# hangxu0304/DeepReduce

Hardware: NVIDIA H100
Metric: ResNet-50 images/sec (whole job, device-timed, max over ranks) (higher is better)
Workload: dtype bf16

## Files before the change

deepreduce_b200/ops/csrc/binding.cpp:

```cpp
#include <ATen/cuda/CUDAContext.h>
#include <c10/cuda/CUDAGuard.h>
#include <c10/cuda/CUDAStream.h>
#include <torch/extension.h>

#include <condition_variable>
#include <deque>
#include <mutex>
#include <thread>

#include "ops.h"

namespace py = pybind11;
using dr::EngineParams;

#define CHECK_CUDA_T(x) TORCH_CHECK((x).is_cuda() && (x).is_contiguous(), #x " must be a contiguous CUDA tensor")

static cudaStream_t cur_stream() { return at::cuda::getCurrentCUDAStream().stream(); }

static void check_last(const char* what) {
  cudaError_t e = cudaGetLastError();
  TORCH_CHECK(e == cudaSuccess, what, ": ", cudaGetErrorString(e));
}

static torch::Tensor bloom_insert(torch::Tensor idx, int64_t k, int64_t m_bits, int64_t seed) {
// ... 144 lines not shown
  const int64_t nb = (n + 127) / 128;
  auto off = torch::empty({nb + 1}, payload.options().dtype(torch::kInt64));
  auto deltas = torch::empty({n}, payload.options().dtype(torch::kInt64));
  dr::launch_bp128_unpack((const uint32_t*)payload.data_ptr<int32_t>(), n, off.data_ptr<int64_t>(),
                          deltas.data_ptr<int64_t>(), cur_stream());
  check_last("delta_bp128_decode");
  return deltas.cumsum(0);
}

static torch::Tensor rle_runs(torch::Tensor idx, int64_t d) {
  CHECK_CUDA_T(idx);
  c10::cuda::CUDAGuard g(idx.device());
  const int64_t n = idx.numel();
  auto o64 = idx.options().dtype(torch::kInt64);
  if (n == 0) return torch::full({1}, d, o64);
  const int64_t nb = (n + 1023) / 1024;
  auto counts = torch::empty({nb}, idx.options().dtype(torch::kInt32));
  auto excl = torch::empty({nb + 1}, idx.options().dtype(torch::kInt32));
  dr::launch_rle_count(idx.data_ptr<int64_t>(), n, (uint32_t*)counts.data_ptr<int32_t>(), (uint32_t*)excl.data_ptr<int32_t>(),
                       cur_stream());
  const int64_t n_runs = excl[nb].item<int32_t>();
  auto start_pos = torch::empty({n_runs}, o64), end_pos = torch::empty({n_runs}, o64);
  auto runs = torch::zeros({2 * n_runs + 1}, o64);
  dr::launch_rle_runs(idx.data_ptr<int64_t>(), n, (const uint32_t*)excl.data_ptr<int32_t>(), start_pos.data_ptr<int64_t>(),
                      end_pos.data_ptr<int64_t>(), n_runs, d, runs.data_ptr<int64_t>(), cur_stream());
  check_last("rle_runs");
  const int64_t last = idx[n - 1].item<int64_t>();
  return (d - 1 - last > 0) ? runs : runs.slice(0, 0, 2 * n_runs);
}

static torch::Tensor rle_indices(torch::Tensor runs) {
  CHECK_CUDA_T(runs);
  c10::cuda::CUDAGuard g(runs.device());
  const int64_t n_pairs = runs.numel() / 2;
  auto o64 = runs.options().dtype(torch::kInt64);
  if (n_pairs == 0) return torch::empty({0}, o64);
  auto pairs = runs.slice(0, 0, 2 * n_pairs).to(torch::kInt64).view({n_pairs, 2});
  auto z = pairs.select(1, 0), o = pairs.select(1, 1);
  auto csum = (z + o).cumsum(0);
  auto run_start = (csum - o).contiguous();
  auto ones_incl = o.cumsum(0);
  auto ones_excl = (ones_incl - o).contiguous();
  const int64_t total = ones_incl[n_pairs - 1].item<int64_t>();
  auto out = torch::empty({total}, o64);
  dr::launch_rle_expand(ones_excl.data_ptr<int64_t>(), run_start.data_ptr<int64_t>(), n_pairs, total, out.data_ptr<int64_t>(),
                        cur_stream());
  check_last("rle_indices");
  return out;
}

static torch::Tensor u8_to_nhwc_norm(torch::Tensor in, std::vector<double> mean, std::vector<double> stdv) {
  CHECK_CUDA_T(in);
  TORCH_CHECK(in.scalar_type() == torch::kUInt8 && in.size(-1) == 3, "expect uint8 [...,3] NHWC");
  c10::cuda::CUDAGuard g(in.device());
  auto out = torch::empty(in.sizes(), in.options().dtype(torch::kBFloat16));
  float m[3] = {(float)mean[0], (float)mean[1], (float)mean[2]};
  float s[3] = {(float)(1.0 / stdv[0]), (float)(1.0 / stdv[1]), (float)(1.0 / stdv[2])};
  dr::launch_u8_to_nhwc_norm(in.data_ptr<uint8_t>(), out.data_ptr(), in.numel() / 3, m, s, cur_stream());
  check_last("u8_to_nhwc_norm");
  return out;
}

namespace at::native {
struct Var;
template <typename scalar_t, typename VarTransform>
void batch_norm_stats_channels_last_cuda_template(const at::Tensor& out_mean, const at::Tensor& out_invstd,
                                                   const at::Tensor& input, double epsilon);
}

static void check_bn_input(const torch::Tensor& x) {
  TORCH_CHECK(x.is_cuda() && x.scalar_type() == torch::kBFloat16 && x.dim() == 4 && x.stride(1) == 1 &&
                  x.is_contiguous(at::MemoryFormat::ChannelsLast),
              "bn: x must be a channels_last bf16 CUDA tensor");
  TORCH_CHECK(x.size(1) % 8 == 0 && x.size(1) <= 8192, "bn: channels must be a multiple of 8, at most 8192");
  TORCH_CHECK(x.numel() < std::numeric_limits<int32_t>::max(), "bn: tensor too large for 32-bit indexing");
}

static void check_chan(const torch::Tensor& t, int64_t C, const char* what) {
  TORCH_CHECK(t.is_cuda() && t.scalar_type() == torch::kFloat32 && t.is_contiguous() && t.numel() == C, "bn: ", what,
              " must be a contiguous float32 CUDA tensor of C elements");
}

static std::vector<torch::Tensor> bn_stats(torch::Tensor x, torch::Tensor running_mean, torch::Tensor running_var,
                                           double momentum, double eps) {
  check_bn_input(x);
  const int64_t C = x.size(1);
  check_chan(running_mean, C, "running_mean");
  check_chan(running_var, C, "running_var");
  const int64_t N = x.numel() / C;
  TORCH_CHECK(N > 1, "bn: expected more than 1 value per channel when training");
  c10::cuda::CUDAGuard g(x.device());
  auto opts = x.options().dtype(torch::kFloat32);
  auto mean = torch::empty({C}, opts), var = torch::empty({C}, opts);
  at::native::batch_norm_stats_channels_last_cuda_template<c10::BFloat16, at::native::Var>(mean, var, x, eps);
  const float bessel = static_cast<float>(static_cast<double>(N) / static_cast<double>(N - 1));
  cudaError_t e = dr::launch_bn_update_stats(mean.data_ptr<float>(), var.data_ptr<float>(), running_mean.data_ptr<float>(),
                                             running_var.data_ptr<float>(), (int)C, (float)momentum, bessel, (float)eps,
                                             cur_stream());
  TORCH_CHECK(e == cudaSuccess, "bn_stats: ", cudaGetErrorString(e));
  return {mean, var};
}

static dr::BnParams bn_params(const std::vector<torch::Tensor>& p, int64_t C) {
  TORCH_CHECK(p.size() == 4, "bn: expected (mean, invstd, weight, bias)");
  const char* names[4] = {"mean", "invstd", "weight", "bias"};
  for (int i = 0; i < 4; ++i) check_chan(p[i], C, names[i]);
  return {p[0].data_ptr<float>(), p[1].data_ptr<float>(), p[2].data_ptr<float>(), p[3].data_ptr<float>()};
}

static void check_like_x(const torch::Tensor& t, const torch::Tensor& x, const char* what) {
  TORCH_CHECK(t.sizes() == x.sizes() && t.strides() == x.strides() && t.scalar_type() == torch::kBFloat16 &&
                  t.device() == x.device(),
              "bn: ", what, " must match x in shape, layout, dtype and device");
}

static std::vector<torch::Tensor> bn_apply(int64_t mode, torch::Tensor x, std::vector<torch::Tensor> p,
                                           c10::optional<torch::Tensor> z, std::vector<torch::Tensor> pz) {
  check_bn_input(x);
  const int64_t C = x.size(1);
  const dr::BnParams px = bn_params(p, C);
  dr::BnParams pzz{};
  const void* zp = nullptr;
  if (mode != 0) {
    TORCH_CHECK(z.has_value(), "bn: mode ", mode, " needs z");
    check_like_x(*z, x, "z");
    zp = z->data_ptr();
    if (mode == 2) pzz = bn_params(pz, C);
  }
  c10::cuda::CUDAGuard g(x.device());
  const int64_t rows = x.numel() / C;
  auto out = torch::empty_like(x);
  auto mask = torch::empty({rows, C / 8}, x.options().dtype(torch::kUInt8));
  cudaError_t e = dr::launch_bn_apply((int)mode, x.data_ptr(), px, zp, pzz, out.data_ptr(), mask.data_ptr(), rows,
                                      (int)C, cur_stream());
  TORCH_CHECK(e == cudaSuccess, "bn_apply: ", cudaGetErrorString(e));
  return {out, mask};
}

static dr::BnParams bn_bwd_params(const std::vector<torch::Tensor>& p, int64_t C) {
  TORCH_CHECK(p.size() == 3, "bn_backward: expected (mean, invstd, weight)");
  const char* names[3] = {"mean", "invstd", "weight"};
  for (int i = 0; i < 3; ++i) check_chan(p[i], C, names[i]);
  return {p[0].data_ptr<float>(), p[1].data_ptr<float>(), p[2].data_ptr<float>(), nullptr};
}

static std::vector<torch::Tensor> bn_backward(int64_t mode, torch::Tensor go, torch::Tensor mask, torch::Tensor x,
                                              std::vector<torch::Tensor> p, c10::optional<torch::Tensor> z,
                                              std::vector<torch::Tensor> pz) {
  TORCH_CHECK(mode >= 0 && mode <= 2, "bn_backward: mode must be 0, 1 or 2");
  check_bn_input(x);
  TORCH_CHECK(go.sizes() == x.sizes() && go.scalar_type() == torch::kBFloat16 && go.device() == x.device() &&
                  go.is_contiguous(at::MemoryFormat::ChannelsLast),
              "bn_backward: go must be a channels_last bf16 tensor of x's shape on x's device");
  const int64_t C = x.size(1), rows = x.numel() / C;
  TORCH_CHECK(mask.is_cuda() && mask.scalar_type() == torch::kUInt8 && mask.is_contiguous() &&
                  mask.numel() == rows * (C / 8) && mask.device() == x.device(),
              "bn_backward: mask must be bn_apply's mask for x");
  c10::cuda::CUDAGuard guard(x.device());
  int block_y = 0, grid_y = 0;
  dr::bn_backward_tree(rows, (int)C, &block_y, &grid_y);
  TORCH_CHECK((int64_t)block_y * grid_y <= rows, "bn_backward: reduction tree wider than the rows");
  const int n_sums = mode == 2 ? 3 : 2;
  auto f32 = x.options().dtype(torch::kFloat32);
  auto sums = torch::empty({n_sums, C}, f32);
  auto staging = grid_y > 1 ? torch::empty({n_sums, grid_y, C}, f32) : torch::Tensor();
  auto dx = torch::empty_like(x), dw = torch::empty({C}, f32), db = torch::empty({C}, f32);
  dr::BnBwd b{};
  b.go = go.data_ptr(); b.mask = mask.data_ptr<uint8_t>(); b.x = x.data_ptr();
  b.px = bn_bwd_params(p, C);
  b.dx = dx.data_ptr(); b.sums = sums.data_ptr<float>(); b.staging = grid_y > 1 ? staging.data_ptr<float>() : nullptr;
  b.dw = dw.data_ptr<float>(); b.db = db.data_ptr<float>();
  std::vector<torch::Tensor> res{dx, dw, db};
  if (mode == 1) {
    auto g = torch::empty_like(x);
    b.g = g.data_ptr();
    res.push_back(g);
  } else if (mode == 2) {
    TORCH_CHECK(z.has_value(), "bn_backward: mode 2 needs z");
    check_like_x(*z, x, "z");
    b.z = z->data_ptr();
    b.pz = bn_bwd_params(pz, C);
    auto dz = torch::empty_like(x), dwz = torch::empty({C}, f32), dbz = torch::empty({C}, f32);
    b.dz = dz.data_ptr(); b.dwz = dwz.data_ptr<float>(); b.dbz = dbz.data_ptr<float>();
    res.insert(res.end(), {dz, dwz, dbz});
  }
  cudaError_t e = dr::launch_bn_backward((int)mode, b, rows, (int)C, cur_stream());
  TORCH_CHECK(e == cudaSuccess, "bn_backward: ", cudaGetErrorString(e));
  return res;
}

struct Engine {
  EngineParams P{};
  int grid = 0;
  int grid_cap = 0;
  int blocks_per_sm = 2;
  int dyn_smem = 64 * 1024;
  int device = 0;

  Engine(int64_t tensors, int64_t tiles, int64_t n_tensors, int64_t n_tiles, int64_t slot_words,
         int64_t payload_words, int64_t grad, int64_t resid, int64_t hist, int64_t hist_total, int64_t sel,
         int64_t tile_count, int64_t barrier, int64_t status, std::vector<int64_t> arenas, int rank, int world) {
    TORCH_CHECK(world <= dr::kMaxWorld && (int)arenas.size() == world, "bad world/arenas");
    P.tensors = reinterpret_cast<const dr::TensorDesc*>(tensors);
    P.tiles = reinterpret_cast<const dr::TileInfo*>(tiles);
    P.n_tensors = (uint32_t)n_tensors; P.n_tiles = (uint32_t)n_tiles;
    P.slot_words = (uint32_t)slot_words; P.payload_words = (uint32_t)payload_words;
    P.grad = reinterpret_cast<float*>(grad); P.resid = reinterpret_cast<float*>(resid);
    P.hist = reinterpret_cast<uint32_t*>(hist); P.hist_total = reinterpret_cast<uint32_t*>(hist_total);
    P.sel = reinterpret_cast<dr::SelState*>(sel);
    P.tile_count = reinterpret_cast<uint32_t*>(tile_count);
    P.barrier = reinterpret_cast<uint32_t*>(barrier); P.status = reinterpret_cast<uint32_t*>(status);
    for (int i = 0; i < world; ++i) P.arena[i] = reinterpret_cast<uint32_t*>(arenas[i]);
    P.rank = rank; P.world = world;
    P.beta = 1.f; P.gamma = 1.f; P.scale = 1.f / world; P.seed = dr::kDefaultSeed; P.policy = 0; P.use_history = 1;
    P.spin_limit = 20u * 1000u * 1000u;
    P.filter_smem_words = (uint32_t)(dyn_smem / 4);
    P.use_tma = 1; P.hist_shift = 23;
    P.shard = 0; P.s2_words = 0; P.s2_cap = 0; P.has_rle = 0; P.mc_arena = nullptr;
    P.peer_timeout_ms = 120000u; P.fault = 0; P.debug_times = nullptr; P.cost_prefix = nullptr; P.deterministic = 0; P.cuts = nullptr; P.cuts_grid = 0;
    cudaGetDevice(&device);
  }

  void configure(double beta, double gamma, double scale, int64_t seed, int policy, int use_history, int64_t spin_limit,
                 int bps, int64_t filter_smem_bytes, int use_tma, int hist_shift) {
    P.beta = (float)beta; P.gamma = (float)gamma; P.scale = (float)scale; P.seed = (uint32_t)seed;
    P.policy = policy; P.use_history = use_history; P.spin_limit = (uint32_t)spin_limit;
    blocks_per_sm = bps; grid = 0;
    dyn_smem = (int)filter_smem_bytes; P.filter_smem_words = (uint32_t)(dyn_smem / 4);
    P.use_tma = use_tma; P.hist_shift = (uint32_t)hist_shift;
  }

  void set_poly(int64_t tensors, int64_t n_poly, int64_t tasks, int64_t n_tasks, int64_t bins, int64_t bucket_val,
                int64_t bucket_pos, int64_t expand_buf, int64_t poly_total) {
    P.poly_tensors = reinterpret_cast<const uint32_t*>(tensors); P.n_poly = (uint32_t)n_poly;
    P.poly_tasks = reinterpret_cast<const uint32_t*>(tasks); P.n_poly_tasks = (uint32_t)n_tasks;
    P.poly_bins = reinterpret_cast<uint32_t*>(bins); P.bucket_val = reinterpret_cast<float*>(bucket_val);
    P.bucket_pos = reinterpret_cast<uint32_t*>(bucket_pos); P.expand_buf = reinterpret_cast<float*>(expand_buf);
    P.poly_total = (uint32_t)poly_total;
  }

  void set_has_rle(int v) { P.has_rle = v; }
  void set_scratch(int64_t pos_mask, int64_t dec_mask, int64_t cand, int64_t cand_cnt) {
    P.pos_mask = reinterpret_cast<uint32_t*>(pos_mask); P.dec_mask = reinterpret_cast<uint32_t*>(dec_mask);
// ... 80 lines not shown
    cudaSetDevice(device);
    while (true) {
      Item it;
      {
        std::unique_lock<std::mutex> l(mu);
        cv.wait(l, [this] { return stop || !q.empty(); });
        if (q.empty()) return;
        it = q.front(); q.pop_front();
      }
      cudaStreamWaitEvent(side, it.ready, 0);
      try {
        it.eng->run_on(it.epoch, dr::kPhAccum, dr::kPhEnd, side);
      } catch (const std::exception& ex) {
        std::lock_guard<std::mutex> l(mu);
        error = ex.what();
      }
      cudaEventRecord(it.done, side);
      {
        std::lock_guard<std::mutex> l(mu);
        ++completed;
      }
      cv_done.notify_all();
    }
  }

  void submit(int bucket, Engine* eng, int64_t epoch) {
    cudaEventRecord(ready_ev[bucket], cur_stream());
    {
      std::lock_guard<std::mutex> l(mu);
      q.push_back(Item{eng, (uint32_t)epoch, ready_ev[bucket], done_ev[bucket]});
      ++submitted;
    }
    cv.notify_one();
  }

  void wait_all() {
    py::gil_scoped_release rel;
    {
      std::unique_lock<std::mutex> l(mu);
      cv_done.wait(l, [this] { return completed == submitted; });
      TORCH_CHECK(error.empty(), "background engine launch failed: ", error);
    }
    for (auto e : done_ev) cudaStreamWaitEvent(cur_stream(), e, 0);
  }
};

static int64_t arena_alloc(int64_t bytes) {
  void* p = dr::arena_alloc((size_t)bytes);
  TORCH_CHECK(p != nullptr, "arena cudaMalloc failed");
  return (int64_t)p;
}
static py::bytes arena_export(int64_t p) {
  dr::ArenaHandle h = dr::arena_export((void*)p);
  return py::bytes((const char*)h.bytes, sizeof(h.bytes));
}
static int64_t arena_import(const std::string& b) {
  TORCH_CHECK(b.size() == sizeof(dr::ArenaHandle), "bad handle");
  dr::ArenaHandle h;
  memcpy(h.bytes, b.data(), sizeof(h.bytes));
  void* p = dr::arena_import(h);
  TORCH_CHECK(p != nullptr, "cudaIpcOpenMemHandle failed (peer access / IPC unavailable)");
  return (int64_t)p;
}
static torch::Tensor arena_as_tensor(int64_t p, int64_t n_words, int64_t device) {
  auto opts = torch::TensorOptions().dtype(torch::kInt32).device(torch::kCUDA, (int)device);
  return torch::from_blob((void*)p, {n_words}, opts);
}

PYBIND11_MODULE(TORCH_EXTENSION_NAME, m) {
  m.def("launch_count", [] { return (int64_t)dr::launch_count(); });
  m.def("bloom_insert", &bloom_insert);
  m.def("bloom_select", &bloom_select);
  m.def("qsgd_encode", &qsgd_encode);
  m.def("qsgd_decode", &qsgd_decode);
  m.def("pack_bits", &pack_bits);
  m.def("unpack_bits", &unpack_bits);
  m.def("polyfit_fit", &polyfit_fit);
  m.def("polyfit_eval", &polyfit_eval);
  m.def("dexp_fit", &dexp_fit);
  m.def("conflict_sets_pick", &conflict_sets_pick);
  m.def("delta_bp128_encode", &delta_bp128_encode);
  m.def("delta_bp128_decode", &delta_bp128_decode);
  m.def("u8_to_nhwc_norm", &u8_to_nhwc_norm);
  m.def("bn_stats", &bn_stats);
  m.def("bn_apply", &bn_apply, py::arg("mode"), py::arg("x"), py::arg("p"), py::arg("z") = py::none(),
        py::arg("pz") = std::vector<torch::Tensor>{});
  m.def("bn_backward", &bn_backward, py::arg("mode"), py::arg("go"), py::arg("mask"), py::arg("x"), py::arg("p"),
        py::arg("z") = py::none(), py::arg("pz") = std::vector<torch::Tensor>{});
  m.def("rle_runs", &rle_runs);
  m.def("rle_indices", &rle_indices);
  m.def("arena_alloc", &arena_alloc);
  m.def("arena_free", [](int64_t p) { dr::arena_free((void*)p); });
  m.def("arena_export", &arena_export);
  m.def("arena_import", &arena_import);
  m.def("arena_close", [](int64_t p) { dr::arena_close((void*)p); });
  m.def("arena_as_tensor", &arena_as_tensor);
  m.def("enable_peer_access", [](std::vector<int> devices) { return dr::arena_enable_peer_access(devices.data(), (int)devices.size()); });
  m.attr("TILE") = dr::kTile;
  m.attr("ARENA_HDR_WORDS") = dr::kArenaHdrWords;
  m.attr("SLOT_HEADER_WORDS") = dr::kSlotHeaderWords;
  m.attr("HIST_BINS") = dr::kHistBins;
  m.attr("NUM_HIST") = dr::kNumHist;
  m.attr("PH_END") = (int)dr::kPhEnd;

  py::class_<Engine>(m, "Engine")
      .def(py::init<int64_t, int64_t, int64_t, int64_t, int64_t, int64_t, int64_t, int64_t, int64_t, int64_t, int64_t,
                    int64_t, int64_t, int64_t, std::vector<int64_t>, int, int>())
      .def("configure", &Engine::configure)
      .def("set_buffers", &Engine::set_buffers)
      .def("set_poly", &Engine::set_poly)
      .def("set_shard", &Engine::set_shard)
      .def("set_has_rle", &Engine::set_has_rle)
      .def("set_scratch", &Engine::set_scratch)
      .def("set_peer_timeout_ms", &Engine::set_peer_timeout_ms)
      .def("set_fault", &Engine::set_fault)
      .def("set_deterministic", &Engine::set_deterministic)
      .def("set_cost_prefix", &Engine::set_cost_prefix)
      .def("set_debug_times", &Engine::set_debug_times)
      .def("set_cuts", &Engine::set_cuts)
      .def("set_grid_cap", &Engine::set_grid_cap)
      .def("set_multicast", &Engine::set_multicast)
      .def("grid", &Engine::get_grid)
      .def("run", &Engine::run);

  py::class_<Scheduler>(m, "Scheduler")
      .def(py::init<int>())
      .def("submit", &Scheduler::submit)
      .def("wait_all", &Scheduler::wait_all)
      .def("shutdown", &Scheduler::shutdown);
}
```

deepreduce_b200/ops/csrc/bn.cu:

```cuda
#include <cuda_bf16.h>

#include <algorithm>

#include "common.cuh"
#include "ops.h"

namespace dr {

namespace {

constexpr int kVec = 8;
constexpr int kApplyThreads = 256;
constexpr int kReduceThreads = 128;

struct ChanParams {
  float m[kVec], inv[kVec], w[kVec], b[kVec];
};

__device__ __forceinline__ void load8(const float* __restrict__ p, float* d) {
  const float4 a = __ldg(reinterpret_cast<const float4*>(p));
  const float4 b = __ldg(reinterpret_cast<const float4*>(p) + 1);
  d[0] = a.x; d[1] = a.y; d[2] = a.z; d[3] = a.w;
  d[4] = b.x; d[5] = b.y; d[6] = b.z; d[7] = b.w;
}

__device__ __forceinline__ void load_params(const BnParams& p, int c, ChanParams& o) {
  load8(p.mean + c, o.m);
  load8(p.invstd + c, o.inv);
  load8(p.weight + c, o.w);
  load8(p.bias + c, o.b);
}

__device__ __forceinline__ float bn_elem(float x, float m, float inv, float w, float b) {
  return __fmaf_rn(__fmul_rn(w, __fsub_rn(x, m)), inv, b);
}

__device__ __forceinline__ __nv_bfloat16 relu_bf16(__nv_bfloat16 v) {
  return __bfloat162float(v) <= 0.f ? __float2bfloat16_rn(0.f) : v;
}

template <int kMode>
__global__ void __launch_bounds__(kApplyThreads) bn_apply_kernel(const __nv_bfloat16* __restrict__ x, BnParams px,
                                                                 const __nv_bfloat16* __restrict__ z, BnParams pz,
                                                                 __nv_bfloat16* __restrict__ out,
                                                                 uint8_t* __restrict__ mask, int64_t rows, int C) {
  const int groups = C / kVec;
  const int rows_per_cta = blockDim.x / groups;
  const int rsub = threadIdx.x / groups;
  if (rsub >= rows_per_cta) return;
  const int c = (threadIdx.x % groups) * kVec;
  ChanParams a;
  load_params(px, c, a);
  ChanParams d;
  if (kMode == 2) load_params(pz, c, d);
  const int64_t step = (int64_t)gridDim.x * rows_per_cta;
#pragma unroll 2
  for (int64_t r = (int64_t)blockIdx.x * rows_per_cta + rsub; r < rows; r += step) {
    const int64_t off = r * C + c;
    const uint4 vx = *reinterpret_cast<const uint4*>(x + off);
    uint4 vz = make_uint4(0, 0, 0, 0);
    if (kMode != 0) vz = *reinterpret_cast<const uint4*>(z + off);
    const __nv_bfloat16* hx = reinterpret_cast<const __nv_bfloat16*>(&vx);
    const __nv_bfloat16* hz = reinterpret_cast<const __nv_bfloat16*>(&vz);
    uint4 vo;
    __nv_bfloat16* ho = reinterpret_cast<__nv_bfloat16*>(&vo);
    unsigned bits = 0;
#pragma unroll
    for (int i = 0; i < kVec; ++i) {
      __nv_bfloat16 y = __float2bfloat16_rn(bn_elem(__bfloat162float(hx[i]), a.m[i], a.inv[i], a.w[i], a.b[i]));
      if (kMode != 0) {
        const __nv_bfloat16 s = kMode == 1 ? hz[i]
                                           : __float2bfloat16_rn(bn_elem(__bfloat162float(hz[i]), d.m[i], d.inv[i], d.w[i], d.b[i]));
        y = __float2bfloat16_rn(__fadd_rn(__bfloat162float(y), __bfloat162float(s)));
      }
      ho[i] = relu_bf16(y);
      bits |= (__bfloat162float(ho[i]) <= 0.f ? 0u : 1u) << i;
    }
    *reinterpret_cast<uint4*>(out + off) = vo;
    mask[r * groups + c / kVec] = (uint8_t)bits;
  }
}

struct BwdTree {
  int block_y, grid_y;
  __host__ __device__ int S() const { return block_y * grid_y; }
  __host__ __device__ int loops(int rows) const { return 1 + (rows - 1) / (S() * kBwdLoads); }
  static constexpr int kBwdLoads = 4;
};

template <int kN>
__device__ __forceinline__ void tree_over_y(float* v, float* sh, int y, int n, int col, int width) {
  for (int off = n / 2; off > 0; off >>= 1) {
#pragma unroll
    for (int i = 0; i < kN; ++i) sh[y * width + col + i] = v[i];
    __syncthreads();
    if (y < off) {
#pragma unroll
      for (int i = 0; i < kN; ++i) v[i] = __fadd_rn(v[i], sh[(y + off) * width + col + i]);
    }
    __syncthreads();
  }
}

struct BwdOut {
  float* sums;
  float* dw; float* db; float* dwz; float* dbz;
  float* staging;
};

__device__ __forceinline__ void bwd_store(const BwdOut& o, int k, int c, int C, float v, const float* invstd,
                                         const float* invstd_z) {
  o.sums[k * C + c] = v;
  if (k == 0) {
    o.db[c] = v;
    if (o.dbz) o.dbz[c] = v;
  } else if (k == 1) {
    o.dw[c] = __fmul_rn(v, invstd[c]);
  } else {
    o.dwz[c] = __fmul_rn(v, invstd_z[c]);
  }
}

__device__ __forceinline__ float masked(__nv_bfloat16 go, unsigned bit) { return bit ? __bfloat162float(go) : 0.f; }

template <int kMode>
__global__ void __launch_bounds__(kReduceThreads) bn_bwd_reduce_kernel(const __nv_bfloat16* __restrict__ go,
                                                                       const uint8_t* __restrict__ mask,
                                                                       const __nv_bfloat16* __restrict__ x,
                                                                       const float* __restrict__ mean,
                                                                       const float* __restrict__ invstd,
                                                                       const __nv_bfloat16* __restrict__ z,
                                                                       const float* __restrict__ mean_z,
                                                                       const float* __restrict__ invstd_z,
                                                                       __nv_bfloat16* __restrict__ g_out, BwdOut o,
                                                                       BwdTree t, int rows, int C) {
  constexpr int kSums = kMode == 2 ? 3 : 2;
  constexpr int L = BwdTree::kBwdLoads;
  extern __shared__ float sh[];
  const int gpc = blockDim.x / t.block_y;
  const int tg = threadIdx.x % gpc, y = threadIdx.x / gpc;
  const int group = blockIdx.x * gpc + tg;
  const bool live = group * kVec < C;
  const int c = live ? group * kVec : 0;
  const int S = t.S();
  float m[kVec], mz[kVec];
#pragma unroll
  for (int i = 0; i < kVec; ++i) {
    m[i] = mean[c + i];
    mz[i] = kMode == 2 ? mean_z[c + i] : 0.f;
  }
  float acc[kSums][L][kVec];
#pragma unroll
  for (int k = 0; k < kSums; ++k)
#pragma unroll
    for (int j = 0; j < L; ++j)
#pragma unroll
      for (int i = 0; i < kVec; ++i) acc[k][j][i] = 0.f;
  const int mgroups = C / kVec;
  int r = blockIdx.y * t.block_y + y;
  const int n_loops = t.loops(rows);
  struct Batch {
    uint4 g[L], x[L], z[L];
    unsigned m[L];
  };
  auto load = [&](Batch& b, int r0) {
#pragma unroll
    for (int j = 0; j < L; ++j) {
      const int rr = r0 + j * S;
      if (live && rr < rows) {
        const int off = rr * C + c;
        b.g[j] = *reinterpret_cast<const uint4*>(go + off);
        b.x[j] = *reinterpret_cast<const uint4*>(x + off);
        if (kMode == 2) b.z[j] = *reinterpret_cast<const uint4*>(z + off);
        b.m[j] = mask[rr * mgroups + group];
      } else {
        b.g[j] = uint4{}; b.x[j] = uint4{}; b.z[j] = uint4{}; b.m[j] = 0;
      }
    }
  };
  Batch cur;
  load(cur, r);
  for (int it = 0; it < n_loops; ++it) {
    Batch nxt;
    load(nxt, r + L * S);
    const unsigned* mb = cur.m;
#pragma unroll
    for (int j = 0; j < L; ++j) {
      const __nv_bfloat16* hg = reinterpret_cast<const __nv_bfloat16*>(&cur.g[j]);
      const __nv_bfloat16* hx = reinterpret_cast<const __nv_bfloat16*>(&cur.x[j]);
      const __nv_bfloat16* hz = reinterpret_cast<const __nv_bfloat16*>(&cur.z[j]);
      uint4 vo;
      __nv_bfloat16* ho = reinterpret_cast<__nv_bfloat16*>(&vo);
#pragma unroll
      for (int i = 0; i < kVec; ++i) {
        const unsigned bit = (mb[j] >> i) & 1u;
        const float g = masked(hg[i], bit);
        if (kMode == 1) ho[i] = bit ? hg[i] : __float2bfloat16_rn(0.f);
        acc[0][j][i] = __fadd_rn(acc[0][j][i], g);
        acc[1][j][i] = __fmaf_rn(__fsub_rn(__bfloat162float(hx[i]), m[i]), g, acc[1][j][i]);
        if (kMode == 2) acc[2][j][i] = __fmaf_rn(__fsub_rn(__bfloat162float(hz[i]), mz[i]), g, acc[2][j][i]);
      }
      if (kMode == 1 && live && r + j * S < rows) *reinterpret_cast<uint4*>(g_out + (r + j * S) * C + c) = vo;
    }
    cur = nxt;
    r += L * S;
  }
#pragma unroll
  for (int k = 0; k < kSums; ++k) {
#pragma unroll
    for (int i = 0; i < kVec; ++i)
#pragma unroll
      for (int j = 1; j < L; ++j) acc[k][0][i] = __fadd_rn(acc[k][0][i], acc[k][j][i]);
    tree_over_y<kVec>(acc[k][0], sh, y, t.block_y, tg * kVec, gpc * kVec);
  }
  if (y != 0 || !live) return;
#pragma unroll
  for (int k = 0; k < kSums; ++k)
#pragma unroll
    for (int i = 0; i < kVec; ++i) {
      if (t.grid_y > 1) o.staging[((size_t)k * t.grid_y + blockIdx.y) * C + c + i] = acc[k][0][i];
      else bwd_store(o, k, c + i, C, acc[k][0][i], invstd, invstd_z);
    }
}

__global__ void bn_bwd_finalize_kernel(BwdOut o, BwdTree t, int n_sums, int C, const float* __restrict__ invstd,
                                       const float* __restrict__ invstd_z) {
  extern __shared__ float sh[];
  const int cols = blockDim.x / t.block_y;
  const int col = threadIdx.x % cols, y = threadIdx.x / cols;
  const int c = blockIdx.x * cols + col;
  for (int k = 0; k < n_sums; ++k) {
    float v = 0.f;
    if (c < C)
      for (int b = y; b < t.grid_y; b += t.block_y) v = __fadd_rn(v, o.staging[((size_t)k * t.grid_y + b) * C + c]);
    tree_over_y<1>(&v, sh, y, t.block_y, col, cols);
    if (y == 0 && c < C) bwd_store(o, k, c, C, v, invstd, invstd_z);
  }
}

struct ElemtChan {
  float m[kVec], f1[kVec], f2[kVec], sdy[kVec];
};

__device__ __forceinline__ void elemt_params(const float* mean, const float* invstd, const float* w, const float* sdy,
                                             const float* sxmu, float norm, int c, ElemtChan& p) {
  float inv[kVec], ww[kVec], sx[kVec];
  load8(mean + c, p.m);
  load8(invstd + c, inv);
  load8(w + c, ww);
  load8(sdy + c, p.sdy);
  load8(sxmu + c, sx);
#pragma unroll
  for (int i = 0; i < kVec; ++i) {
    p.f1[i] = __fmul_rn(__fmul_rn(__fmul_rn(inv[i], inv[i]), sx[i]), norm);
    p.f2[i] = __fmul_rn(ww[i], inv[i]);
  }
}

__device__ __forceinline__ __nv_bfloat16 elemt(float g, float x, const ElemtChan& p, int i, float norm) {
  const float a = __fmaf_rn(-p.sdy[i], norm, g);
  return __float2bfloat16_rn(__fmul_rn(__fmaf_rn(-p.f1[i], __fsub_rn(x, p.m[i]), a), p.f2[i]));
}

struct ElemtArgs {
  const float *mean, *invstd, *weight, *sums;
  const float *mean_z, *invstd_z, *weight_z;
};

template <int kMode>
__global__ void __launch_bounds__(kApplyThreads) bn_bwd_elemt_kernel(const __nv_bfloat16* __restrict__ g_in,
                                                                     const uint8_t* __restrict__ mask,
                                                                     const __nv_bfloat16* __restrict__ x,
                                                                     const __nv_bfloat16* __restrict__ z, ElemtArgs a,
                                                                     __nv_bfloat16* __restrict__ dx,
                                                                     __nv_bfloat16* __restrict__ dz, float norm,
                                                                     int64_t rows, int C) {
  const int groups = C / kVec;
  const int rows_per_cta = blockDim.x / groups;
  const int rsub = threadIdx.x / groups;
  if (rsub >= rows_per_cta) return;
  const int c = (threadIdx.x % groups) * kVec;
  ElemtChan p;
  elemt_params(a.mean, a.invstd, a.weight, a.sums, a.sums + C, norm, c, p);
  ElemtChan q;
  if (kMode == 2) elemt_params(a.mean_z, a.invstd_z, a.weight_z, a.sums, a.sums + 2 * C, norm, c, q);
  const int64_t step = (int64_t)gridDim.x * rows_per_cta;
#pragma unroll 2
  for (int64_t r = (int64_t)blockIdx.x * rows_per_cta + rsub; r < rows; r += step) {
    const int64_t off = r * C + c;
    const uint4 vg = *reinterpret_cast<const uint4*>(g_in + off);
    const uint4 vx = *reinterpret_cast<const uint4*>(x + off);
    uint4 vz = make_uint4(0, 0, 0, 0);
    if (kMode == 2) vz = *reinterpret_cast<const uint4*>(z + off);
    const unsigned mb = kMode == 1 ? 0xffu : mask[r * groups + c / kVec];
    const __nv_bfloat16* hg = reinterpret_cast<const __nv_bfloat16*>(&vg);
    const __nv_bfloat16* hx = reinterpret_cast<const __nv_bfloat16*>(&vx);
    const __nv_bfloat16* hz = reinterpret_cast<const __nv_bfloat16*>(&vz);
    uint4 vo, vd;
    __nv_bfloat16* ho = reinterpret_cast<__nv_bfloat16*>(&vo);
    __nv_bfloat16* hd = reinterpret_cast<__nv_bfloat16*>(&vd);
#pragma unroll
    for (int i = 0; i < kVec; ++i) {
      const float g = masked(hg[i], (mb >> i) & 1u);
      ho[i] = elemt(g, __bfloat162float(hx[i]), p, i, norm);
      if (kMode == 2) hd[i] = elemt(g, __bfloat162float(hz[i]), q, i, norm);
    }
    *reinterpret_cast<uint4*>(dx + off) = vo;
    if (kMode == 2) *reinterpret_cast<uint4*>(dz + off) = vd;
  }
}

__global__ void bn_update_stats_kernel(const float* __restrict__ mean, float* __restrict__ var_invstd,
                                       float* __restrict__ running_mean, float* __restrict__ running_var, int C,
                                       float momentum, float bessel, float eps) {
  const int c = blockIdx.x * blockDim.x + threadIdx.x;
  if (c >= C) return;
  const float m = mean[c], v = var_invstd[c];
  const float unbiased_var = v * bessel;
  running_mean[c] = m * momentum + (1 - momentum) * running_mean[c];
  running_var[c] = unbiased_var * momentum + (1 - momentum) * running_var[c];
  var_invstd[c] = rsqrtf(v + eps);
}

template <typename K>
cudaError_t rows_grid(K kernel, int64_t rows, int C, int& grid, int& threads) {
  const int groups = C / kVec;
  const int rows_per_cta = groups >= kApplyThreads ? 1 : kApplyThreads / groups;
  threads = groups * rows_per_cta;
  int per_sm = 0;
  cudaError_t e = cudaOccupancyMaxActiveBlocksPerMultiprocessor(&per_sm, kernel, threads, 0);
  if (e != cudaSuccess) return e;
  int64_t g = (rows + rows_per_cta - 1) / rows_per_cta;
  const int64_t cap = (int64_t)(per_sm > 0 ? per_sm : 1) * sm_count();
  grid = (int)(g > cap ? cap : g);
  return cudaSuccess;
}

template <int kMode>
cudaError_t launch_apply(const void* x, const BnParams& px, const void* z, const BnParams& pz, void* out, void* mask,
                         int64_t rows, int C, cudaStream_t st) {
  if (rows == 0) return cudaSuccess;
  int grid = 0, threads = 0;
  cudaError_t e = rows_grid(bn_apply_kernel<kMode>, rows, C, grid, threads);
  if (e != cudaSuccess) return e;
  count_launch();
  bn_apply_kernel<kMode><<<grid, threads, 0, st>>>(reinterpret_cast<const __nv_bfloat16*>(x), px,
                                                   reinterpret_cast<const __nv_bfloat16*>(z), pz,
                                                   reinterpret_cast<__nv_bfloat16*>(out),
                                                   reinterpret_cast<uint8_t*>(mask), rows, C);
  return cudaGetLastError();
}

int last_pow2(unsigned n) {
  n |= n >> 1; n |= n >> 2; n |= n >> 4; n |= n >> 8; n |= n >> 16;
  return std::max<int>(1, (int)(n - (n >> 1)));
}

BwdTree bwd_tree(int rows, int C) {
  const int block_x = std::min(last_pow2((unsigned)C), 32);
  const int block_y = std::min(last_pow2((unsigned)((rows + 15) / 16)), 512 / block_x);
  int grid_y = std::min((rows + block_y * 16 - 1) / (block_y * 16), 128);
  if (grid_y < 8) grid_y = 1;
  return {block_y, grid_y};
}

template <int kMode>
cudaError_t launch_bwd_reduce(const BnBwd& b, const BwdTree& t, const BwdOut& o, int rows, int C, cudaStream_t st) {
  const int groups = C / kVec;
  const int gpc = std::min(groups, std::max(1, kReduceThreads / t.block_y));
  const dim3 grid((groups + gpc - 1) / gpc, t.grid_y);
  const int threads = gpc * t.block_y;
  count_launch();
  bn_bwd_reduce_kernel<kMode><<<grid, threads, threads * kVec * sizeof(float), st>>>(
      reinterpret_cast<const __nv_bfloat16*>(b.go), b.mask, reinterpret_cast<const __nv_bfloat16*>(b.x), b.px.mean,
      b.px.invstd, reinterpret_cast<const __nv_bfloat16*>(b.z), b.pz.mean, b.pz.invstd,
      reinterpret_cast<__nv_bfloat16*>(b.g), o, t, rows, C);
  return cudaGetLastError();
}

template <int kMode>
cudaError_t launch_bwd_elemt(const BnBwd& b, const ElemtArgs& a, int64_t rows, int C, cudaStream_t st) {
  int grid = 0, threads = 0;
  cudaError_t e = rows_grid(bn_bwd_elemt_kernel<kMode>, rows, C, grid, threads);
  if (e != cudaSuccess) return e;
  const float norm = (float)(1.0 / (double)rows);
  count_launch();
  bn_bwd_elemt_kernel<kMode><<<grid, threads, 0, st>>>(
      reinterpret_cast<const __nv_bfloat16*>(kMode == 1 ? b.g : b.go), b.mask,
      reinterpret_cast<const __nv_bfloat16*>(b.x), reinterpret_cast<const __nv_bfloat16*>(b.z), a,
      reinterpret_cast<__nv_bfloat16*>(b.dx), reinterpret_cast<__nv_bfloat16*>(b.dz), norm, rows, C);
  return cudaGetLastError();
}

template <int kMode>
cudaError_t launch_backward(const BnBwd& b, int64_t rows64, int C, cudaStream_t st) {
  const int rows = (int)rows64;
  const BwdTree t = bwd_tree(rows, C);
  const BwdOut o{b.sums, b.dw, b.db, b.dwz, b.dbz, b.staging};
  cudaError_t e = launch_bwd_reduce<kMode>(b, t, o, rows, C, st);
  if (e != cudaSuccess) return e;
  if (t.grid_y > 1) {
    const int cols = std::max(1, 512 / t.block_y);
    const int threads = cols * t.block_y;
    count_launch();
    bn_bwd_finalize_kernel<<<(C + cols - 1) / cols, threads, threads * sizeof(float), st>>>(
        o, t, kMode == 2 ? 3 : 2, C, b.px.invstd, b.pz.invstd);
    e = cudaGetLastError();
    if (e != cudaSuccess) return e;
  }
  const ElemtArgs a{b.px.mean, b.px.invstd, b.px.weight, b.sums, b.pz.mean, b.pz.invstd, b.pz.weight};
  return launch_bwd_elemt<kMode>(b, a, rows64, C, st);
}

}

void bn_backward_tree(int64_t rows, int C, int* block_y, int* grid_y) {
  const BwdTree t = bwd_tree((int)rows, C);
  *block_y = t.block_y;
  *grid_y = t.grid_y;
}

cudaError_t launch_bn_backward(int mode, const BnBwd& b, int64_t rows, int C, cudaStream_t st) {
  if (rows == 0) return cudaSuccess;
  switch (mode) {
    case 0: return launch_backward<0>(b, rows, C, st);
    case 1: return launch_backward<1>(b, rows, C, st);
    case 2: return launch_backward<2>(b, rows, C, st);
    default: return cudaErrorInvalidValue;
  }
}

cudaError_t launch_bn_update_stats(const float* mean, float* var_invstd, float* running_mean, float* running_var, int C,
                                   float momentum, float bessel, float eps, cudaStream_t st) {
  count_launch();
  bn_update_stats_kernel<<<(C + 255) / 256, 256, 0, st>>>(mean, var_invstd, running_mean, running_var, C, momentum,
                                                          bessel, eps);
  return cudaGetLastError();
}

cudaError_t launch_bn_apply(int mode, const void* x, const BnParams& px, const void* z, const BnParams& pz, void* out,
                            void* mask, int64_t rows, int C, cudaStream_t st) {
  switch (mode) {
    case 0: return launch_apply<0>(x, px, z, pz, out, mask, rows, C, st);
    case 1: return launch_apply<1>(x, px, z, pz, out, mask, rows, C, st);
    case 2: return launch_apply<2>(x, px, z, pz, out, mask, rows, C, st);
    default: return cudaErrorInvalidValue;
  }
}

}
```

deepreduce_b200/ops/csrc/ops.h:

```cpp
#pragma once
#include <cuda_runtime.h>
#include <stdint.h>

#include "plan.h"

namespace dr {

int engine_max_grid(int blocks_per_sm, int dyn_smem_bytes);
cudaError_t engine_launch(const EngineParams& P, int grid, int blocks_per_sm, int dyn_smem_bytes, cudaStream_t stream);
void count_launch(int n);
long long launch_count();

void launch_bloom_insert(const int64_t* idx, int64_t n, uint32_t* filter, uint32_t n_hash, uint32_t m_bits,
                         uint32_t seed, cudaStream_t st);
void launch_bloom_count(const uint32_t* filter, uint32_t d, uint32_t n_hash, uint32_t m_bits, uint32_t seed,
                        uint32_t* tile_counts, uint32_t* tile_excl, cudaStream_t st);
void launch_bloom_emit(const uint32_t* filter, uint32_t d, uint32_t n_hash, uint32_t m_bits, uint32_t seed,
                       const uint32_t* tile_excl, int64_t* out, uint32_t limit, cudaStream_t st);
void launch_qsgd_encode(const float* v, int64_t K, int bucket, int q, uint32_t seed, void* lvl, bool i16, float* norms,
                        cudaStream_t st);
void launch_qsgd_decode(const void* lvl, bool i16, const float* norms, int64_t K, int bucket, int q, float* out,
                        cudaStream_t st);
void launch_pack_bits(const int64_t* vals, int64_t n, int bits, uint32_t* out, int64_t n_words, cudaStream_t st);
void launch_unpack_bits(const uint32_t* in, int64_t n_words, int64_t n, int bits, int64_t* out, cudaStream_t st);
void launch_polyfit_fit(const float* y, const int* seg_off, const int* seg_len, int n_seg, int degree, float* coeffs,
                        cudaStream_t st);
void launch_polyfit_eval(const float* coeffs, const int* seg_off, const int* seg_len, int n_seg, int degree,
                         int64_t total, float* out, cudaStream_t st);
cudaError_t launch_conflict_sets_pick(const uint32_t* set_off, const uint32_t* members, uint32_t* last, uint32_t n_sets, uint32_t n_pos,
                                      uint32_t K, uint32_t pseed, uint32_t* chosen_out, cudaStream_t st);
void launch_dexp_fit(const float* y, int64_t K, double* out_abpq, cudaStream_t st);
void launch_bp128_widths(const int64_t* idx, int64_t n, uint32_t* widths, cudaStream_t st);
void launch_bp128_pack(const int64_t* idx, int64_t n, const uint32_t* widths, const int64_t* word_off, uint32_t* out,
                       cudaStream_t st);
void launch_bp128_unpack(const uint32_t* in, int64_t n, int64_t* word_off, int64_t* deltas, cudaStream_t st);
void launch_rle_count(const int64_t* idx, int64_t n, uint32_t* counts, uint32_t* excl, cudaStream_t st);
void launch_rle_runs(const int64_t* idx, int64_t n, const uint32_t* excl, int64_t* start_pos, int64_t* end_pos,
                     int64_t n_runs, int64_t d, int64_t* runs, cudaStream_t st);
void launch_rle_expand(const int64_t* ones_excl, const int64_t* run_start, int64_t n_runs, int64_t total, int64_t* out,
                       cudaStream_t st);

struct ArenaHandle { unsigned char bytes[64]; };
void* arena_alloc(size_t bytes);
void arena_free(void* p);
ArenaHandle arena_export(void* p);
void* arena_import(const ArenaHandle& h);
void arena_close(void* p);
int arena_enable_peer_access(const int* devices, int n);
void launch_u8_to_nhwc_norm(const uint8_t* in, void* out_bf16, int64_t n_pix, const float* mean, const float* inv_std,
                            cudaStream_t st);

struct BnParams { const float* mean; const float* invstd; const float* weight; const float* bias; };
cudaError_t launch_bn_update_stats(const float* mean, float* var_invstd, float* running_mean, float* running_var, int C,
                                   float momentum, float bessel, float eps, cudaStream_t st);
cudaError_t launch_bn_apply(int mode, const void* x, const BnParams& px, const void* z, const BnParams& pz, void* out,
                            void* mask, int64_t rows, int C, cudaStream_t st);
struct BnBwd {
  const void* go; const uint8_t* mask; const void* x; const void* z;
  BnParams px, pz;
  void* dx; void* dz; void* g;
  float* sums; float* staging; float* dw; float* db; float* dwz; float* dbz;
};
void bn_backward_tree(int64_t rows, int C, int* block_y, int* grid_y);
cudaError_t launch_bn_backward(int mode, const BnBwd& b, int64_t rows, int C, cudaStream_t st);

}
```

Before: 5041.

## Add custom Welford BN stats kernel fused with running-stat update

Replaces PyTorch's channels_last batch-norm stats template with a custom two-stage Welford reduction. It reads 8-channel bf16 vectors with software-prefetched loads, merges partials in shared memory, and writes mean, invstd and running stats in the final stage. This folds the separate running-stat update kernel into the reduction, and the vectorised reduction tree is shared with the backward kernel. The PyTorch path is kept behind a flag, and the new reduction order may shift numerics slightly.

```diff
diff --git a/deepreduce_b200/ops/csrc/binding.cpp b/deepreduce_b200/ops/csrc/binding.cpp
--- a/deepreduce_b200/ops/csrc/binding.cpp
+++ b/deepreduce_b200/ops/csrc/binding.cpp
@@ -250,7 +250,7 @@
 }
 
 static std::vector<torch::Tensor> bn_stats(torch::Tensor x, torch::Tensor running_mean, torch::Tensor running_var,
-                                           double momentum, double eps) {
+                                           double momentum, double eps, bool torch_kernel) {
   check_bn_input(x);
   const int64_t C = x.size(1);
   check_chan(running_mean, C, "running_mean");
@@ -259,14 +259,25 @@
   TORCH_CHECK(N > 1, "bn: expected more than 1 value per channel when training");
   c10::cuda::CUDAGuard g(x.device());
   auto opts = x.options().dtype(torch::kFloat32);
-  auto mean = torch::empty({C}, opts), var = torch::empty({C}, opts);
-  at::native::batch_norm_stats_channels_last_cuda_template<c10::BFloat16, at::native::Var>(mean, var, x, eps);
+  auto mean = torch::empty({C}, opts), invstd = torch::empty({C}, opts);
   const float bessel = static_cast<float>(static_cast<double>(N) / static_cast<double>(N - 1));
-  cudaError_t e = dr::launch_bn_update_stats(mean.data_ptr<float>(), var.data_ptr<float>(), running_mean.data_ptr<float>(),
-                                             running_var.data_ptr<float>(), (int)C, (float)momentum, bessel, (float)eps,
-                                             cur_stream());
+  int block_y = 0, grid_y = 0;
+  dr::bn_row_tree(N, (int)C, &block_y, &grid_y);
+  cudaError_t e;
+  if (!torch_kernel && (int64_t)block_y * grid_y <= N) {
+    auto staging = grid_y > 1 ? torch::empty({(2 * C + 1) * grid_y}, opts) : torch::Tensor();
+    const dr::BnStats s{x.data_ptr(), mean.data_ptr<float>(), invstd.data_ptr<float>(), running_mean.data_ptr<float>(),
+                        running_var.data_ptr<float>(), grid_y > 1 ? staging.data_ptr<float>() : nullptr,
+                        (float)momentum, bessel, (float)eps};
+    e = dr::launch_bn_stats(s, N, (int)C, cur_stream());
+  } else {
+    at::native::batch_norm_stats_channels_last_cuda_template<c10::BFloat16, at::native::Var>(mean, invstd, x, eps);
+    e = dr::launch_bn_update_stats(mean.data_ptr<float>(), invstd.data_ptr<float>(), running_mean.data_ptr<float>(),
+                                   running_var.data_ptr<float>(), (int)C, (float)momentum, bessel, (float)eps,
+                                   cur_stream());
+  }
   TORCH_CHECK(e == cudaSuccess, "bn_stats: ", cudaGetErrorString(e));
-  return {mean, var};
+  return {mean, invstd};
 }
 
 static dr::BnParams bn_params(const std::vector<torch::Tensor>& p, int64_t C) {
@@ -326,7 +337,7 @@
               "bn_backward: mask must be bn_apply's mask for x");
   c10::cuda::CUDAGuard guard(x.device());
   int block_y = 0, grid_y = 0;
-  dr::bn_backward_tree(rows, (int)C, &block_y, &grid_y);
+  dr::bn_row_tree(rows, (int)C, &block_y, &grid_y);
   TORCH_CHECK((int64_t)block_y * grid_y <= rows, "bn_backward: reduction tree wider than the rows");
   const int n_sums = mode == 2 ? 3 : 2;
   auto f32 = x.options().dtype(torch::kFloat32);
@@ -573,7 +584,8 @@
   m.def("delta_bp128_encode", &delta_bp128_encode);
   m.def("delta_bp128_decode", &delta_bp128_decode);
   m.def("u8_to_nhwc_norm", &u8_to_nhwc_norm);
-  m.def("bn_stats", &bn_stats);
+  m.def("bn_stats", &bn_stats, py::arg("x"), py::arg("running_mean"), py::arg("running_var"), py::arg("momentum"),
+        py::arg("eps"), py::arg("torch_kernel") = false);
   m.def("bn_apply", &bn_apply, py::arg("mode"), py::arg("x"), py::arg("p"), py::arg("z") = py::none(),
         py::arg("pz") = std::vector<torch::Tensor>{});
   m.def("bn_backward", &bn_backward, py::arg("mode"), py::arg("go"), py::arg("mask"), py::arg("x"), py::arg("p"),
diff --git a/deepreduce_b200/ops/csrc/bn.cu b/deepreduce_b200/ops/csrc/bn.cu
--- a/deepreduce_b200/ops/csrc/bn.cu
+++ b/deepreduce_b200/ops/csrc/bn.cu
@@ -81,12 +81,170 @@
   }
 }
 
-struct BwdTree {
+struct RowTree {
   int block_y, grid_y;
   __host__ __device__ int S() const { return block_y * grid_y; }
-  __host__ __device__ int loops(int rows) const { return 1 + (rows - 1) / (S() * kBwdLoads); }
-  static constexpr int kBwdLoads = 4;
+  __host__ __device__ int loops(int rows) const { return 1 + (rows - 1) / (S() * kLoads); }
+  static constexpr int kLoads = 4;
 };
+
+constexpr int kStatsThreads = 256;
+
+__device__ __forceinline__ void welford_update(float x, float inv, float valid, float& mean, float& m2n) {
+  const float d0 = __fsub_rn(x, mean);
+  mean = __fmaf_rn(d0, inv, mean);
+  const float d1 = __fsub_rn(x, mean);
+  m2n = __fmaf_rn(__fmul_rn(d0, d1), valid, m2n);
+}
+
+template <int kN, bool kFuseNew>
+__device__ __forceinline__ void welford_merge(int& n, float* mean, float* m2n, int n_new, const float* mean_new,
+                                              const float* m2n_new) {
+  const float fn = (float)n, fn_new = (float)n_new;
+  const float factor = __frcp_rn((float)max(1, n + n_new));
+#pragma unroll
+  for (int i = 0; i < kN; ++i) {
+    const float d = __fsub_rn(mean[i], mean_new[i]);
+    const float s = kFuseNew ? __fmaf_rn(mean_new[i], fn_new, __fmul_rn(mean[i], fn))
+                             : __fmaf_rn(mean[i], fn, __fmul_rn(mean_new[i], fn_new));
+    mean[i] = __fmul_rn(s, factor);
+    const float u = __fmul_rn(__fmul_rn(__fmul_rn(d, d), fn_new), fn);
+    m2n[i] = __fadd_rn(m2n[i], __fmaf_rn(u, factor, m2n_new[i]));
+  }
+  n += n_new;
+}
+
+template <int kN>
+struct WelfordSlots {
+  float* mean; float* m2n; int* count;
+  __device__ WelfordSlots(float* sh, int slots)
+      : mean(sh), m2n(sh + slots * kN), count(reinterpret_cast<int*>(sh + 2 * slots * kN)) {}
+  __device__ void put(int s, int n, const float* m, const float* q) const {
+#pragma unroll
+    for (int i = 0; i < kN; ++i) { mean[s * kN + i] = m[i]; m2n[s * kN + i] = q[i]; }
+    count[s] = n;
+  }
+  template <bool kFuseNew>
+  __device__ void merge_from(int s, int& n, float* m, float* q) const {
+    float mn[kN], qn[kN];
+#pragma unroll
+    for (int i = 0; i < kN; ++i) { mn[i] = mean[s * kN + i]; qn[i] = m2n[s * kN + i]; }
+    welford_merge<kN, kFuseNew>(n, m, q, count[s], mn, qn);
+  }
+  static size_t bytes(int slots) { return (size_t)slots * (2 * kN * sizeof(float) + sizeof(int)); }
+};
+
+template <int kN>
+__device__ __forceinline__ void welford_tree_over_y(const WelfordSlots<kN>& sl, bool part, int y, int block_y, int base,
+                                                    int stride, int& n, float* mean, float* m2n) {
+  for (int off = block_y / 2; off > 0; off >>= 1) {
+    if (part && y < 2 * off) sl.put(base + y * stride, n, mean, m2n);
+    __syncthreads();
+    if (part && y < off) sl.template merge_from<false>(base + (y + off) * stride, n, mean, m2n);
+    __syncthreads();
+  }
+}
+
+struct StatsOut {
+  float* mean; float* invstd; float* running_mean; float* running_var;
+  float* st_mean; float* st_m2n; int* st_count;
+  float momentum, bessel, eps;
+};
+
+__device__ __forceinline__ void stats_store(const StatsOut& o, int c, int n, float mean, float m2n) {
+  const float var = __fdiv_rn(m2n, (float)n);
+  const float keep = __fsub_rn(1.f, o.momentum);
+  o.mean[c] = mean;
+  o.invstd[c] = rsqrtf(__fadd_rn(var, o.eps));
+  o.running_mean[c] = __fmaf_rn(mean, o.momentum, __fmul_rn(o.running_mean[c], keep));
+  o.running_var[c] = __fmaf_rn(__fmul_rn(var, o.bessel), o.momentum, __fmul_rn(o.running_var[c], keep));
+}
+
+__global__ void __launch_bounds__(kStatsThreads) bn_stats_kernel(const __nv_bfloat16* __restrict__ x, StatsOut o,
+                                                                 RowTree t, int rows, int C) {
+  constexpr int L = RowTree::kLoads;
+  constexpr int kAhead = 4;
+  extern __shared__ float sh[];
+  const int gpc = blockDim.x / (L * t.block_y);
+  const int g = threadIdx.x % gpc, j = (threadIdx.x / gpc) % L, y = threadIdx.x / (gpc * L);
+  const int group = blockIdx.x * gpc + g;
+  const bool live = group * kVec < C;
+  const int c = live ? group * kVec : 0;
+  const int S = t.S();
+  const int n_loops = t.loops(rows);
+  const int r0 = blockIdx.y * t.block_y + y + j * S;
+  const int rstep = L * S;
+  float mean[kVec], m2n[kVec];
+#pragma unroll
+  for (int i = 0; i < kVec; ++i) mean[i] = m2n[i] = 0.f;
+  int n = 0;
+  auto load = [&](uint4* b, int i0) {
+#pragma unroll
+    for (int u = 0; u < kAhead; ++u) {
+      const int r = r0 + (i0 + u) * rstep;
+      b[u] = live && i0 + u < n_loops && r < rows ? *reinterpret_cast<const uint4*>(x + (size_t)r * C + c) : uint4{};
+    }
+  };
+  uint4 cur[kAhead];
+  load(cur, 0);
+  for (int i0 = 0; i0 < n_loops; i0 += kAhead) {
+    uint4 nxt[kAhead];
+    load(nxt, i0 + kAhead);
+#pragma unroll
+    for (int u = 0; u < kAhead; ++u) {
+      const int i = i0 + u;
+      if (i >= n_loops) break;
+      const bool valid = r0 + i * rstep < rows;
+      const float inv = valid ? __frcp_rn((float)(i + 1)) : 0.f;
+      const float fv = valid ? 1.f : 0.f;
+      n += valid;
+      const __nv_bfloat16* hx = reinterpret_cast<const __nv_bfloat16*>(&cur[u]);
+#pragma unroll
+      for (int k = 0; k < kVec; ++k) welford_update(__bfloat162float(hx[k]), inv, fv, mean[k], m2n[k]);
+    }
+#pragma unroll
+    for (int u = 0; u < kAhead; ++u) cur[u] = nxt[u];
+  }
+  const WelfordSlots<kVec> sl(sh, blockDim.x);
+  sl.put(threadIdx.x, n, mean, m2n);
+  __syncthreads();
+  if (j == 0) {
+#pragma unroll
+    for (int a = 1; a < L; ++a) sl.merge_from<true>(threadIdx.x + a * gpc, n, mean, m2n);
+  }
+  __syncthreads();
+  welford_tree_over_y<kVec>(sl, j == 0, y, t.block_y, g, gpc * L, n, mean, m2n);
+  if (j != 0 || y != 0 || !live) return;
+  if (t.grid_y == 1) {
+#pragma unroll
+    for (int i = 0; i < kVec; ++i) stats_store(o, c + i, n, mean[i], m2n[i]);
+    return;
+  }
+#pragma unroll
+  for (int i = 0; i < kVec; ++i) {
+    o.st_mean[(size_t)blockIdx.y * C + c + i] = mean[i];
+    o.st_m2n[(size_t)blockIdx.y * C + c + i] = m2n[i];
+  }
+  if (group == 0) o.st_count[blockIdx.y] = n;
+}
+
+__global__ void bn_stats_finalize_kernel(StatsOut o, RowTree t, int C) {
+  extern __shared__ float sh[];
+  const int cols = blockDim.x / t.block_y;
+  const int col = threadIdx.x % cols, y = threadIdx.x / cols;
+  const int c = blockIdx.x * cols + col;
+  int n = 0;
+  float mean = 0.f, m2n = 0.f;
+  if (c < C)
+    for (int b = y; b < t.grid_y; b += t.block_y) {
+      const float mb = o.st_mean[(size_t)b * C + c], qb = o.st_m2n[(size_t)b * C + c];
+      welford_merge<1, false>(n, &mean, &m2n, o.st_count[b], &mb, &qb);
+    }
+  const WelfordSlots<1> sl(sh, blockDim.x);
+  welford_tree_over_y<1>(sl, true, y, t.block_y, col, cols, n, &mean, &m2n);
+  if (y == 0 && c < C) stats_store(o, c, n, mean, m2n);
+}
+
 
 template <int kN>
 __device__ __forceinline__ void tree_over_y(float* v, float* sh, int y, int n, int col, int width) {
@@ -133,9 +291,9 @@
                                                                        const float* __restrict__ mean_z,
                                                                        const float* __restrict__ invstd_z,
                                                                        __nv_bfloat16* __restrict__ g_out, BwdOut o,
-                                                                       BwdTree t, int rows, int C) {
+                                                                       RowTree t, int rows, int C) {
   constexpr int kSums = kMode == 2 ? 3 : 2;
-  constexpr int L = BwdTree::kBwdLoads;
+  constexpr int L = RowTree::kLoads;
   extern __shared__ float sh[];
   const int gpc = blockDim.x / t.block_y;
   const int tg = threadIdx.x % gpc, y = threadIdx.x / gpc;
@@ -223,7 +381,7 @@
     }
 }
 
-__global__ void bn_bwd_finalize_kernel(BwdOut o, BwdTree t, int n_sums, int C, const float* __restrict__ invstd,
+__global__ void bn_bwd_finalize_kernel(BwdOut o, RowTree t, int n_sums, int C, const float* __restrict__ invstd,
                                        const float* __restrict__ invstd_z) {
   extern __shared__ float sh[];
   const int cols = blockDim.x / t.block_y;
@@ -356,7 +514,7 @@
   return std::max<int>(1, (int)(n - (n >> 1)));
 }
 
-BwdTree bwd_tree(int rows, int C) {
+RowTree row_tree(int rows, int C) {
   const int block_x = std::min(last_pow2((unsigned)C), 32);
   const int block_y = std::min(last_pow2((unsigned)((rows + 15) / 16)), 512 / block_x);
   int grid_y = std::min((rows + block_y * 16 - 1) / (block_y * 16), 128);
@@ -365,7 +523,7 @@
 }
 
 template <int kMode>
-cudaError_t launch_bwd_reduce(const BnBwd& b, const BwdTree& t, const BwdOut& o, int rows, int C, cudaStream_t st) {
+cudaError_t launch_bwd_reduce(const BnBwd& b, const RowTree& t, const BwdOut& o, int rows, int C, cudaStream_t st) {
   const int groups = C / kVec;
   const int gpc = std::min(groups, std::max(1, kReduceThreads / t.block_y));
   const dim3 grid((groups + gpc - 1) / gpc, t.grid_y);
@@ -395,7 +553,7 @@
 template <int kMode>
 cudaError_t launch_backward(const BnBwd& b, int64_t rows64, int C, cudaStream_t st) {
   const int rows = (int)rows64;
-  const BwdTree t = bwd_tree(rows, C);
+  const RowTree t = row_tree(rows, C);
   const BwdOut o{b.sums, b.dw, b.db, b.dwz, b.dbz, b.staging};
   cudaError_t e = launch_bwd_reduce<kMode>(b, t, o, rows, C, st);
   if (e != cudaSuccess) return e;
@@ -412,10 +570,31 @@
   return launch_bwd_elemt<kMode>(b, a, rows64, C, st);
 }
 
-}
-
-void bn_backward_tree(int64_t rows, int C, int* block_y, int* grid_y) {
-  const BwdTree t = bwd_tree((int)rows, C);
+cudaError_t launch_stats(const BnStats& s, int rows, int C, cudaStream_t st) {
+  const RowTree t = row_tree(rows, C);
+  const int grid_y = t.grid_y;
+  const StatsOut o{s.mean, s.invstd, s.running_mean, s.running_var,
+                   s.staging, s.staging + (size_t)grid_y * C, reinterpret_cast<int*>(s.staging + 2 * (size_t)grid_y * C),
+                   s.momentum, s.bessel, s.eps};
+  const int groups = C / kVec;
+  const int gpc = std::min(groups, std::max(1, kStatsThreads / (RowTree::kLoads * t.block_y)));
+  const int threads = gpc * RowTree::kLoads * t.block_y;
+  count_launch();
+  bn_stats_kernel<<<dim3((groups + gpc - 1) / gpc, grid_y), threads, WelfordSlots<kVec>::bytes(threads), st>>>(
+      reinterpret_cast<const __nv_bfloat16*>(s.x), o, t, rows, C);
+  cudaError_t e = cudaGetLastError();
+  if (e != cudaSuccess || grid_y == 1) return e;
+  const int cols = std::max(1, 512 / t.block_y);
+  const int fthreads = cols * t.block_y;
+  count_launch();
+  bn_stats_finalize_kernel<<<(C + cols - 1) / cols, fthreads, WelfordSlots<1>::bytes(fthreads), st>>>(o, t, C);
+  return cudaGetLastError();
+}
+
+}
+
+void bn_row_tree(int64_t rows, int C, int* block_y, int* grid_y) {
+  const RowTree t = row_tree((int)rows, C);
   *block_y = t.block_y;
   *grid_y = t.grid_y;
 }
@@ -430,6 +609,11 @@
   }
 }
 
+cudaError_t launch_bn_stats(const BnStats& s, int64_t rows, int C, cudaStream_t st) {
+  if (rows == 0) return cudaSuccess;
+  return launch_stats(s, (int)rows, C, st);
+}
+
 cudaError_t launch_bn_update_stats(const float* mean, float* var_invstd, float* running_mean, float* running_var, int C,
                                    float momentum, float bessel, float eps, cudaStream_t st) {
   count_launch();
diff --git a/deepreduce_b200/ops/csrc/ops.h b/deepreduce_b200/ops/csrc/ops.h
--- a/deepreduce_b200/ops/csrc/ops.h
+++ b/deepreduce_b200/ops/csrc/ops.h
@@ -51,6 +51,14 @@
                             cudaStream_t st);
 
 struct BnParams { const float* mean; const float* invstd; const float* weight; const float* bias; };
+void bn_row_tree(int64_t rows, int C, int* block_y, int* grid_y);
+struct BnStats {
+  const void* x;
+  float* mean; float* invstd; float* running_mean; float* running_var;
+  float* staging;
+  float momentum, bessel, eps;
+};
+cudaError_t launch_bn_stats(const BnStats& s, int64_t rows, int C, cudaStream_t st);
 cudaError_t launch_bn_update_stats(const float* mean, float* var_invstd, float* running_mean, float* running_var, int C,
                                    float momentum, float bessel, float eps, cudaStream_t st);
 cudaError_t launch_bn_apply(int mode, const void* x, const BnParams& px, const void* z, const BnParams& pz, void* out,
@@ -61,7 +69,6 @@
   void* dx; void* dz; void* g;
   float* sums; float* staging; float* dw; float* db; float* dwz; float* dbz;
 };
-void bn_backward_tree(int64_t rows, int C, int* block_y, int* grid_y);
 cudaError_t launch_bn_backward(int mode, const BnBwd& b, int64_t rows, int C, cudaStream_t st);
 
 }
```

Result: faster. 5675 (median of 6 runs) (+12.6%).
